# wakensky/parameter_server

Hardware: AMD Instinct MI355X
Metric: aggregated kv-pairs/s (device-resident), N-way sparse push merge at 1/2/4/8 GPU (higher is better)
Workload: dtype f32; 1 GPU; cfg2: 8 pushes x 131072 sorted unique uint64 keys + f32 values, 10% shared keys (U=956,827); 64 such (channel,time) aggregates per GPU per step; global_batch=64, input_layout=arena, parallelism=key-range shards evenDivide(1); worker-sliced ingress, no data-path collective

## Files before the change

include/psg.h:

```cpp
#ifndef PSG_H_
#define PSG_H_

#include <stddef.h>
#include <stdint.h>

#ifdef __cplusplus
extern "C" {
#endif

#define PSG_ABI_VERSION 1
#define PSG_MAX_VALUE_ARRAYS 4

typedef enum psg_status {
  PSG_OK = 0,
  PSG_ERR_ARG = -1,
  PSG_ERR_UNMATCHED = -2,
  PSG_ERR_RANGE = -3,
  PSG_ERR_NO_TIME = -4,
  PSG_ERR_OOM = -5,
  PSG_ERR_DEVICE = -6,
  PSG_ERR_UNSORTED = -7,
  PSG_ERR_SIZE = -8,
  PSG_ERR_CHANNEL = -9,
  PSG_ERR_EMPTY_KEYS = -10,
  PSG_ERR_SIGNATURE = -11
} psg_status;

typedef enum psg_dtype { PSG_F32 = 0, PSG_F64 = 1 } psg_dtype;

#define PSG_SERIAL_MATCH 0u
#define PSG_PARALLEL_MATCH 1u
#define PSG_HOLD_BUFFERS 0x100u
#define PSG_FORM_PACKED 0x1000u
#define PSG_FORM_UNIFORM 0x2000u
#define PSG_PART_SEARCH 0x4000u
#define PSG_PART_STREAM 0x8000u
#define PSG_GROUP32 0x10000u
#define PSG_GROUP64 0x20000u
#define PSG_NO_DENSE 0x40000u
#define PSG_NO_ZERO_COPY 0x80000u
#define PSG_NO_INDEX 0x100000u
#define PSG_FORM_CURSOR 0x400000u
#define PSG_NO_CURSOR 0x800000u
#define PSG_STATIC_KEYS 0x200000u

int psg_abi_version(void);
const char* psg_status_string(int status);
const char* psg_last_error(void);
int psg_device_count(int* n);

typedef struct psg_ctx psg_ctx;

int psg_create(int device, int dtype, unsigned flags, psg_ctx** out);
int psg_destroy(psg_ctx* ctx);
int psg_set_match_flags(psg_ctx* ctx, unsigned flags);
int psg_set_flush_pushes(psg_ctx* ctx, int n);

int psg_key_union(psg_ctx* ctx, int chl, const uint64_t* keys, size_t n);
int psg_key_union_batch(psg_ctx* ctx, int chl, const uint64_t* const* keys, const size_t* n,
                        int npush);
int psg_key_size(psg_ctx* ctx, int chl, size_t* n);
int psg_key_copy(psg_ctx* ctx, int chl, size_t off, size_t n, uint64_t* out);
int psg_find_range(psg_ctx* ctx, int chl, uint64_t kb, uint64_t ke,
                   size_t* lo, size_t* hi);
int psg_value_assign(psg_ctx* ctx, int chl, const void* vals, size_t n);
int psg_value_size(psg_ctx* ctx, int chl, size_t* n);
int psg_value_copy(psg_ctx* ctx, int chl, size_t off, size_t n, void* out);

int psg_push(psg_ctx* ctx, int chl, int time, uint64_t kb, uint64_t ke,
             const uint64_t* keys, size_t n, int m, const void* const* vals);

int psg_push_compressed(psg_ctx* ctx, int chl, int time, uint64_t kb, uint64_t ke,
                        const void* ckeys, size_t ckeys_bytes, int m,
                        const void* const* cvals, const size_t* cvals_bytes);

#define PSG_KC_SIG 1u
// ... 17 lines not shown
                 const uint64_t* keys_dev, size_t n, int m, const void* const* vals_dev,
                 size_t slice, void* stream);
int psg_pull_dev(psg_ctx* ctx, int chl, const uint64_t* keys_dev, size_t n, void* out_dev,
                 unsigned long long* matched_dev, void* stream);
int psg_dev_status(psg_ctx* ctx);

typedef struct psg_merge_job {
  const uint64_t* keys;
  uint64_t nslots;
  int npush;
  const uint64_t* const* push_keys;
  const void* const* push_vals;
  const uint64_t* push_n;
  void* const* out;
} psg_merge_job;

typedef struct psg_plan psg_plan;

int psg_plan_create(int device, int dtype, int m, unsigned flags,
                    const psg_merge_job* jobs, int njobs, psg_plan** out);
int psg_plan_max_push(void);
int psg_plan_run(psg_plan* plan, void* stream);
int psg_plan_run_stage(psg_plan* plan, int stage, void* stream);
int psg_plan_matched(psg_plan* plan, uint64_t* matched);
#define PSG_KERNEL_TILE 0
#define PSG_KERNEL_TILE64 1
#define PSG_KERNEL_PACKED 2
#define PSG_KERNEL_DENSE 3
#define PSG_KERNEL_CURSOR 4
#define PSG_KERNEL_PACKED_CURSOR 5
int psg_plan_form(psg_plan* plan, int* form);
int psg_plan_bytes(psg_plan* plan, uint64_t* bytes, uint64_t* kv_pairs);
int psg_plan_index_info(psg_plan* plan, uint64_t* index_bytes, uint64_t* marked_tiles);
int psg_plan_destroy(psg_plan* plan);

int psg_gather_dev(int dtype, const uint64_t* dkeys, uint64_t nd,
                   const void* dvals, const uint64_t* req, uint64_t nreq,
                   void* out, unsigned long long* matched, void* stream);

int psg_key_union_dev(const uint64_t* a, uint64_t na, const uint64_t* b,
                      uint64_t nb, uint64_t* out, uint64_t* nout,
                      void* stream);

typedef struct psg_nway psg_nway;
int psg_nway_max_push(void);
int psg_nway_create(int device, int dtype, int m, unsigned flags, int npush,
                    const uint64_t* const* keys, const uint64_t* n, const void* const* vals,
                    uint64_t* out_keys, void* const* out_vals, psg_nway** out);
int psg_nway_create_batch(int device, int dtype, int m, unsigned flags, int nmerge,
                          const int* npush, const uint64_t* const* keys, const uint64_t* n,
                          const void* const* vals, uint64_t* const* out_keys,
                          void* const* out_vals, psg_nway** out);
int psg_nway_run(psg_nway* u, void* stream);
int psg_nway_count_dev(psg_nway* u, unsigned long long** nout);
int psg_nway_result(psg_nway* u, uint64_t* nout);
int psg_nway_bytes(psg_nway* u, uint64_t* bytes, uint64_t* kv_pairs);
int psg_nway_destroy(psg_nway* u);

#define PSG_COMM_ID_BYTES 128
typedef struct psg_comm psg_comm;
int psg_comm_unique_id(uint8_t* id);
int psg_comm_init(int device, int nranks, const uint8_t* id, int rank,
                  psg_comm** out);
int psg_comm_destroy(psg_comm* comm);
int psg_comm_init_loopback(int device, int nranks, psg_comm** out);

// ... 205 lines not shown
```

parameter_server_amd/_lib.py:

```python
from __future__ import annotations

import ctypes as C
import os

_HERE = os.path.dirname(os.path.abspath(__file__))
LIB_PATH = os.environ.get("PSG_LIB_PATH") or os.path.join(_HERE, "libpsg.so")

PSG_OK = 0
PSG_ERR_ARG = -1
PSG_ERR_UNMATCHED = -2
PSG_ERR_RANGE = -3
PSG_ERR_NO_TIME = -4
PSG_ERR_OOM = -5
PSG_ERR_DEVICE = -6
PSG_ERR_UNSORTED = -7
PSG_ERR_SIZE = -8
PSG_ERR_CHANNEL = -9
PSG_ERR_EMPTY_KEYS = -10
PSG_ERR_SIGNATURE = -11
PSG_KC_SIG = 1
PSG_KC_KEYS = 2
PSG_KC_ERASE = 4
PSG_MAX_SIG_LEN = 2048
PSG_NO_SLICE = (1 << 64) - 1

PSG_F32 = 0
PSG_F64 = 1
PSG_SERIAL_MATCH = 0
PSG_PARALLEL_MATCH = 1
PSG_HOLD_BUFFERS = 0x100
PSG_FORM_PACKED = 0x1000
PSG_FORM_UNIFORM = 0x2000
PSG_PART_SEARCH = 0x4000
PSG_PART_STREAM = 0x8000
PSG_GROUP32 = 0x10000
PSG_GROUP64 = 0x20000
PSG_NO_DENSE = 0x40000
PSG_NO_ZERO_COPY = 0x80000
PSG_NO_INDEX = 0x100000
PSG_STATIC_KEYS = 0x200000
PSG_FORM_CURSOR = 0x400000
PSG_NO_CURSOR = 0x800000
(PSG_KERNEL_TILE, PSG_KERNEL_TILE64, PSG_KERNEL_PACKED, PSG_KERNEL_DENSE, PSG_KERNEL_CURSOR,
 PSG_KERNEL_PACKED_CURSOR) = range(6)
MAX_VALUE_ARRAYS = 4
MB_STAGES = ("sort", "run_length", "localize", "count_keys", "times", "logit", "trans_times")
PSG_LOSS_LOGIT = 0
(PSG_MB_SORTED_KEY, PSG_MB_SORTED_POS, PSG_MB_UNIQ_KEY, PSG_MB_KEY_CNT, PSG_MB_NEW_OFFSET,
 PSG_MB_NEW_INDEX, PSG_MB_NEW_VALUE, PSG_MB_POS, PSG_MB_NEG, PSG_MB_XW, PSG_MB_TAU, PSG_MB_LOSS,
 PSG_MB_GRAD, PSG_MB_RUN_START, PSG_MB_REMAPPED, PSG_MB_ROW_OF, PSG_MB_SCRATCH) = range(17)
PSG_AUC_BY_KEY, PSG_AUC_AS_WRITTEN = 0, 1
(PSG_MB_DARLING_DUAL, PSG_MB_DARLING_CUR_W, PSG_MB_DARLING_DELTA, PSG_MB_DARLING_ACTIVE,
 PSG_MB_DARLING_DELTA_W) = range(32, 37)
PSG_MB_OFFSET, PSG_MB_INDEX, PSG_MB_VALUE, PSG_MB_Y = range(24, 28)
PSG_TEXT_ADFEA, PSG_TEXT_LIBSVM = 4, 5

_u64 = C.c_uint64
_sz = C.c_size_t
_p = C.c_void_p
_pu64 = C.POINTER(C.c_uint64)
_psz = C.POINTER(C.c_size_t)


class MergeJob(C.Structure):

    _fields_ = [
        ("keys", _p),
        ("nslots", _u64),
        ("npush", C.c_int),
        ("push_keys", C.POINTER(_p)),
        ("push_vals", C.POINTER(_p)),
        ("push_n", _pu64),
        ("out", C.POINTER(_p)),
    ]

# ... 26 lines not shown
    "psg_set_flush_pushes": (C.c_int, [_p, C.c_int]),
    "psg_set_match_flags": (C.c_int, [_p, C.c_uint]),
    "psg_key_union": (C.c_int, [_p, C.c_int, _p, _sz]),
    "psg_key_size": (C.c_int, [_p, C.c_int, _psz]),
    "psg_key_copy": (C.c_int, [_p, C.c_int, _sz, _sz, _p]),
    "psg_find_range": (C.c_int, [_p, C.c_int, _u64, _u64, _psz, _psz]),
    "psg_value_assign": (C.c_int, [_p, C.c_int, _p, _sz]),
    "psg_value_size": (C.c_int, [_p, C.c_int, _psz]),
    "psg_value_copy": (C.c_int, [_p, C.c_int, _sz, _sz, _p]),
    "psg_push": (C.c_int, [_p, C.c_int, C.c_int, _u64, _u64, _p, _sz, C.c_int,
                           C.POINTER(_p)]),
    "psg_push_cached": (C.c_int, [_p, C.c_int, C.c_int, C.c_int, _u64, _u64, C.c_uint,
                                  C.c_uint32, _p, _sz, C.c_int, _p, _sz]),
    "psg_key_cache_clear": (C.c_int, [_p, C.c_int]),
    "psg_push_compressed": (C.c_int, [_p, C.c_int, C.c_int, _u64, _u64, _p, _sz, C.c_int,
                                      _p, _p]),
    "psg_key_cache_bytes": (C.c_int, [_p, C.c_int, _psz]),
    "psg_received_shape": (C.c_int, [_p, C.c_int, C.POINTER(C.c_int), _psz, _psz]),
    "psg_received": (C.c_int, [_p, C.c_int, C.c_int, C.POINTER(_p)]),
    "psg_gather": (C.c_int, [_p, C.c_int, _p, _sz, _p, _psz]),
    "psg_push_dev": (C.c_int, [_p, C.c_int, C.c_int, _u64, _u64, _p, _sz, C.c_int,
                               C.POINTER(_p), _sz, _p]),
    "psg_pull_dev": (C.c_int, [_p, C.c_int, _p, _sz, _p, _p, _p]),
    "psg_dev_status": (C.c_int, [_p]),
    "psg_plan_create": (C.c_int, [C.c_int, C.c_int, C.c_int, C.c_uint,
                                  C.POINTER(MergeJob), C.c_int, C.POINTER(_p)]),
    "psg_plan_max_push": (C.c_int, []),
    "psg_plan_run": (C.c_int, [_p, _p]),
    "psg_plan_run_stage": (C.c_int, [_p, C.c_int, _p]),
    "psg_plan_matched": (C.c_int, [_p, _pu64]),
    "psg_plan_bytes": (C.c_int, [_p, _pu64, _pu64]),
    "psg_plan_form": (C.c_int, [_p, C.POINTER(C.c_int)]),
    "psg_plan_index_info": (C.c_int, [_p, _pu64, _pu64]),
    "psg_plan_destroy": (C.c_int, [_p]),
    "psg_gather_dev": (C.c_int, [C.c_int, _p, _u64, _p, _p, _u64, _p, _p, _p]),
    "psg_key_union_dev": (C.c_int, [_p, _u64, _p, _u64, _p, _pu64, _p]),
    "psg_shard_bounds": (C.c_int, [_sz, _pu64]),
    "psg_slice_dev": (C.c_int, [_p, _u64, _u64, _u64, _p, C.c_int, _p, _p]),
    "psg_crc32c_dev": (C.c_int, [_p, _p, _u64, _u64, _p, _p, _p]),
    "psg_snappy_uncompress_dev": (C.c_int, [_p, _p, _u64, _p, _p, _p, _p]),
    "psg_snappy_uncompressed_length": (C.c_int, [_p, _sz, _psz]),
    "psg_freq_resize": (C.c_int, [_p, C.c_int, C.c_int, C.c_int]),
    "psg_freq_clear": (C.c_int, [_p, C.c_int]),
    "psg_freq_empty": (C.c_int, [_p, C.c_int, C.POINTER(C.c_int)]),
    "psg_freq_insert": (C.c_int, [_p, C.c_int, _p, _p, _sz]),
    "psg_freq_query": (C.c_int, [_p, C.c_int, _p, _sz, C.c_int, _p, _psz]),
    "psg_freq_insert_dev": (C.c_int, [_p, C.c_int, _p, _p, _sz, _p]),
    "psg_freq_query_scratch_bytes": (_sz, [_sz]),
    "psg_freq_query_dev": (C.c_int, [_p, C.c_int, _p, _sz, C.c_int, _p, _p, _p, _p]),
    "psg_freq_table": (C.c_int, [_p, C.c_int, _p, _sz]),
    "psg_freq_table_assign": (C.c_int, [_p, C.c_int, _p, _sz]),
    "psg_comm_unique_id": (C.c_int, [_p]),
    "psg_comm_init": (C.c_int, [C.c_int, C.c_int, _p, C.c_int, C.POINTER(_p)]),
    "psg_comm_destroy": (C.c_int, [_p]),
    "psg_comm_init_loopback": (C.c_int, [C.c_int, C.c_int, C.POINTER(_p)]),
    "psg_exchange_create": (C.c_int, [_p, C.c_int, C.c_int, C.c_int, _p, _p, _p,
                                      C.POINTER(_p)]),
    "psg_exchange_run": (C.c_int, [_p, _p]),
    "psg_exchange_recv": (C.c_int, [_p, C.POINTER(_p), _p, _pu64, _p, _pu64]),
    "psg_exchange_destroy": (C.c_int, [_p]),
    "psg_exchange_status": (C.c_int, [_p, _pu64]),
    "psg_exchange_create_local": (C.c_int, [C.c_int, C.c_int, C.c_int, C.c_int, C.c_int, _p,
                                            _p, _p, C.POINTER(_p)]),
    "psg_exchange_set_direct": (C.c_int, [_p, C.c_int]),
    "psg_exchange_send_layout": (C.c_int, [_p, C.POINTER(_p), _p, _p]),
    "psg_key_union_batch": (C.c_int, [_p, C.c_int, _p, _p, C.c_int]),
# ... 120 lines not shown
```

parameter_server_amd/csrc/psg_internal.h:

```cpp
#pragma once

#include <hip/hip_runtime.h>
#include <stdint.h>

namespace psg {

constexpr int kMaxPush = 4096;
constexpr int kMaxM = 4;
constexpr int kTileSlots = 1024;
#ifndef PSG_PACK_TS
#define PSG_PACK_TS 2048
#endif
constexpr int kPackTileSlots = PSG_PACK_TS;
constexpr int kWideSlots = 2048;

constexpr uint32_t kFlagParallel = 1u;
constexpr uint32_t kFlagCont = 2u;
constexpr uint32_t kFlagLastTile = 4u;

enum PartMode : uint32_t { kSearch = 0, kStream = 1 };
constexpr uint32_t kStreamChunk = 512;

struct JobDev {
  const uint64_t* dkeys;
// ... 28 lines not shown
  const uint64_t* dpos;
  const uint32_t* bt;
};

struct CursorJob {
  const uint64_t* dkeys;
  uint64_t nslots;
  const uint64_t* const* pkeys;
  const void* const* pvals;
  const uint64_t* pn;
  void* const* out;
  unsigned long long* fail;
  uint32_t* seg;
  const uint32_t* bt;
  uint32_t np, ntiles, flags;
  uint32_t kr;
};
struct CursorChunk {
  uint32_t job, t0, t1;
};
constexpr int kCursorPushes = 32;
hipError_t launch_aggregate_cursor(int dtype, int m, int kr, const CursorJob* d_jobs,
                                   const CursorChunk* d_chunks, uint32_t nchunks, uint32_t* bx,
                                   hipStream_t stream);

struct DenseCheck {
  const uint64_t* keys;
  uint64_t n;
  const uint64_t* D;
  uint64_t nd;
  unsigned long long* out;
};

hipError_t launch_partition(const JobDev* d_jobs, const uint32_t* d_split_item_job,
                            uint32_t nsplit_items, const uint64_t* d_items,
                            uint32_t nitems, hipStream_t stream, bool xcd = false);
hipError_t launch_aggregate_tile(int dtype, int m, const TileDesc* d_tiles, uint32_t ntiles,
                                 int form, hipStream_t stream);
uint32_t bucket_index_words(uint32_t tile_slots);
hipError_t launch_bucket_index(const TileDesc* d_tiles, uint32_t ntiles, uint32_t tile_slots,
                               uint32_t* out, unsigned long long* nmarked,
                               hipStream_t stream);
constexpr int kPackCursorPushes = 256;
hipError_t launch_aggregate_tile_packed(int dtype, int m, const TileDesc* d_tiles,
                                        uint32_t ntiles, hipStream_t stream,
                                        const CursorChunk* d_chunks = nullptr,
                                        uint32_t nchunks = 0, uint32_t* bx = nullptr);
hipError_t launch_aggregate_dense(int dtype, int m, const TileDesc* d_tiles, uint32_t ntiles,
                                  hipStream_t stream);
hipError_t launch_dense_check(const DenseCheck* checks, uint32_t nchecks, const uint64_t* items,
                              uint64_t nitems, hipStream_t stream);
hipError_t launch_gather(int dtype, const uint64_t* dkeys, uint64_t nd,
                         const void* dvals, const uint64_t* req, uint64_t nreq,
                         void* out, unsigned long long* matched,
                         hipStream_t stream);
hipError_t launch_pull(int dtype, const uint64_t* dkeys, uint64_t nd, const void* dvals,
                       const uint64_t* req, uint64_t nreq, void* out, unsigned long long* matched,
                       unsigned long long* ctl, unsigned long long* unsorted_total,
                       hipStream_t stream);
struct IntakeArgs {
  const void* src[kMaxM + 1];
  void* dst[kMaxM + 1];
  uint64_t len[kMaxM + 1];
  uint32_t esz[kMaxM + 1];
  uint32_t n = 0;
  const uint64_t* claim_keys = nullptr;
  const uint64_t* D = nullptr;
  uint64_t nclaim = 0;
  unsigned long long* bad = nullptr;
// ... 137 lines not shown
```

parameter_server_amd/csrc/psg_jobimage.cc:

```cpp
#include "psg_jobimage.h"

#include <algorithm>
#include <cmath>
#include <cstring>

#include "psg_host.h"

namespace psg {
namespace {

constexpr double kStreamBelow = 24.0;
constexpr double kPackBelow = 16.0;


uint64_t search_groups(uint64_t nt) { return (nt + 64) / 64; }
uint64_t stream_chunks(uint64_t n) { return (n + kStreamChunk - 1) / kStreamChunk; }
uint64_t split_blocks(uint64_t nt, uint64_t np) { return (std::max(nt + 1, np) + 255) / 256; }

}

int JobImage::plan(const JobSpec* jobs, size_t njobs, int dt, int mm, bool idx) {
  if (njobs > (1ull << 27)) return fail(PSG_ERR_ARG, "too many jobs");
  dtype = dt;
  m = mm;
// ... 132 lines not shown
  L.marked = off;
  if (use_index()) off += 256;
  L.sitems = off;
  off = align_up(off + 4 * (size_t)nsplit, 256);
  L.items = off;
  off = align_up(off + 8 * (size_t)nitems, 256);
  L.cjobs = off;
  if (cursor) off = align_up(off + sizeof(CursorJob) * njobs, 256);
  L.chunks = off;
  if (chunked) off = align_up(off + sizeof(CursorChunk) * nchunks, 256);
  L.zero = off;
  size_t fail_cur = off;
  uint64_t npall = 0;
  for (const JobInfo& I : info) npall += I.np;
  off = align_up(off + 8 * npall, 256);
  L.bx = off;
  if (chunked) off = align_up(off + 4 * (size_t)bxs * ((size_t)nchunks + 1), 256);
  L.zero_end = off;
  L.job.resize(njobs);
  for (size_t j = 0; j < njobs; ++j) {
    const size_t np = info[j].np, nt = info[j].ntiles;
    JobLayout::Job& o = L.job[j];
    o.pk = off; off = align_up(off + 8 * np, 64);
    o.pv = off; off = align_up(off + 8 * np * m, 64);
    o.pn = off; off = align_up(off + 8 * np, 64);
    o.out = off; off = align_up(off + 8 * m, 64);
    o.fail = fail_cur; fail_cur += 8 * np;
    o.seg = off; off = align_up(off + 4 * (nt + 1) * np, 256);
    o.split = off;
    if (info[j].has_split) off = align_up(off + 8 * (nt + 1), 256);
    o.dpos = off;
    if (jobs[j].dense) off = align_up(off + 8 * np, 256);
  }
  L.total = off;
}

bool JobImage::same_shape(const JobSpec* jobs, const void* base) {
  shape.clear();
  if (index || cursor || pcursor) return false;
  const JobLayout& L = lay;
  shape.insert(shape.end(), {(uint64_t)h.size(), tile, (uint64_t)m, (uint64_t)dtype,
                             (uint64_t)pack, (uint64_t)wide, (uint64_t)(uintptr_t)base, L.total,
                             L.tiles, L.zero, nitems, nsplit, ntiles});
  for (size_t j = 0; j < h.size(); ++j) {
    const JobSpec& s = jobs[j];
    const JobDev& d = h[j];
    const JobLayout::Job& o = L.job[j];
    shape.insert(shape.end(), {(uint64_t)info[j].np, s.nslots, (uint64_t)(uintptr_t)s.keys,
                               (uint64_t)s.flags, (uint64_t)s.dense, (uint64_t)d.mode,
                               (uint64_t)d.segq, (uint64_t)d.segb, o.pk, o.pv, o.pn, o.out,
                               o.fail, o.seg, o.split, o.dpos});
    if (d.mode == kStream) shape.insert(shape.end(), info[j].pn.begin(), info[j].pn.end());
  }
  return shape == last_shape;
}

void JobImage::keep_shape() {
  last_shape.swap(shape);
  shape.clear();
}

int JobImage::fill(const JobSpec* jobs, char* img, const void* dev, bool same) {
  const JobLayout& L = lay;
  char* base = (char*)dev;
  const size_t njobs = h.size();
  if (L.zero_end > L.zero) memset(img + L.zero, 0, L.zero_end - L.zero);
  if (use_index()) memset(img + L.marked, 0, 8);
  TileDesc* htiles = (TileDesc*)(img + L.tiles);
  uint32_t* hsitems = (uint32_t*)(img + L.sitems);
  uint64_t* hitems = (uint64_t*)(img + L.items);
  const uint32_t* bt = use_index() ? (const uint32_t*)(base + L.index) : nullptr;
  uint64_t tcur = 0, icur = 0, scur = 0;
  for (size_t j = 0; j < njobs; ++j) {
    const JobSpec& s = jobs[j];
    JobInfo& I = info[j];
    const JobLayout::Job& o = L.job[j];
    const uint32_t np = I.np, nt = I.ntiles;
    uint64_t* hk = (uint64_t*)(img + o.pk);
    uint64_t* hv = (uint64_t*)(img + o.pv);
    for (uint32_t p = 0; p < np; ++p) {
      const uint32_t c = I.slot[p];
      hk[p] = (uint64_t)s.pkeys[c];
      for (int i = 0; i < m; ++i) hv[(size_t)p * m + i] = (uint64_t)s.pvals[(size_t)c * m + i];
    }
    if (np) memcpy(img + o.pn, I.pn.data(), 8 * np);
    if (s.dense) {
      uint64_t* hd = (uint64_t*)(img + o.dpos);
      uint32_t* hs = (uint32_t*)(img + o.seg);
      for (uint32_t p = 0; p < np; ++p) {
        const uint64_t dp = s.dpos[I.slot[p]], n = I.pn[p];
        hd[p] = dp;
        for (uint32_t t = 0; t <= nt; ++t) {
          const uint64_t edge = (uint64_t)t * tile;
          const uint64_t v = edge <= dp ? 0 : std::min<uint64_t>(edge - dp, n);
          hs[(size_t)t * np + p] = (uint32_t)v;
        }
      }
    }
    memcpy(img + o.out, s.out.data(), 8 * m);
    JobDev& d = h[j];
    d.dkeys = s.keys;
    d.pkeys = (const uint64_t* const*)(base + o.pk);
    d.pn = (const uint64_t*)(base + o.pn);
    d.seg = (uint32_t*)(base + o.seg);
    d.fail = (unsigned long long*)(base + o.fail);
    d.split = I.has_split ? (uint64_t*)(base + o.split) : nullptr;
    I.seg = d.seg;
    I.fail = d.fail;
    if (same) continue;
    for (uint32_t b = 0; b < I.nsplit; ++b) hsitems[scur++] = (uint32_t)j;
    if (I.nitems && d.mode == kSearch) {
      const uint64_t ng = search_groups(nt);
      for (uint64_t g = 0; g < ng; ++g)
        for (uint32_t p = 0; p < np; ++p)
          hitems[icur++] = (uint64_t)j << 37 | (uint64_t)p << 24 | g;
    } else if (I.nitems) {
      for (uint32_t p = 0; p < np; ++p) {
        const uint64_t nc = stream_chunks(I.pn[p]);
        for (uint64_t c = 0; c < nc; ++c)
          hitems[icur++] = (uint64_t)j << 37 | (uint64_t)p << 24 | c;
      }
    }
    for (uint32_t t = 0; t < nt; ++t) {
      TileDesc& T = htiles[tcur];
      const uint64_t slot0 = (uint64_t)t * tile;
      T.dk = s.keys + slot0;
      T.seg = d.seg + (size_t)t * d.segb;
      T.pkeys = d.pkeys;
      T.pvals = (const void* const*)(base + o.pv);
      T.pn = d.pn;
      T.out = (void* const*)(base + o.out);
      T.fail = d.fail;
      T.slot0 = slot0;
// ... 53 lines not shown
```

parameter_server_amd/csrc/psg_jobimage.h:

```cpp
#pragma once

#include <stddef.h>
#include <stdint.h>
#include <vector>

#include "psg_internal.h"

namespace psg {

inline size_t align_up(size_t x, size_t a) { return (x + a - 1) / a * a; }

struct JobSpec {
  const uint64_t* keys;
  uint64_t nslots;
  std::vector<const uint64_t*> pkeys;
  std::vector<const void*> pvals;
  std::vector<uint64_t> pn;
  std::vector<void*> out;
  uint32_t flags;
  bool dense = false;
  std::vector<uint64_t> dpos;
};

struct JobInfo {
  uint32_t np = 0, ntiles = 0;
  std::vector<uint64_t> pn;
  std::vector<uint32_t> slot;
  uint32_t ncaller = 0;
  uint32_t* seg = nullptr;
  uint32_t segq = 1;
  unsigned long long* fail = nullptr;
  uint32_t kr = 0;
  uint32_t nch = 0, ch0 = 0;
  uint32_t nitems = 0, nsplit = 0;
  bool has_split = false;
};

struct JobLayout {
  static constexpr size_t jobs = 0;
  size_t tiles = 0;
  size_t index = 0;
  size_t marked = 0;
  size_t sitems = 0;
  size_t items = 0;
  size_t cjobs = 0;
  size_t chunks = 0;
  size_t zero = 0, bx = 0, zero_end = 0;
  struct Job { size_t pk, pv, pn, out, fail, seg, split, dpos; };
  std::vector<Job> job;
  size_t total = 0;
  uint32_t iw = 0;
};

struct JobImage {
  int knob_part = -1, knob_pack = -1, knob_wide = -1, knob_cursor = -1;

  int dtype = 0, m = 1;
  bool index = false;
  bool pack = false;
  bool wide = false;
  bool dense = false;
  bool cursor = false;
  bool pcursor = false;
  uint32_t tile = kTileSlots;
  uint32_t bxs = 32;
  uint32_t nchunks = 0;
  uint32_t ckr = 3;
  uint32_t ntiles = 0, nitems = 0, nsplit = 0;
  bool all_search = false;
  std::vector<JobDev> h;
  std::vector<JobInfo> info;
  JobLayout lay;
  bool use_index() const { return index && !dense; }

  std::vector<uint64_t> last_shape, shape;

  int plan(const JobSpec* jobs, size_t njobs, int dtype, int m, bool index);
  void layout(const JobSpec* jobs, uint32_t iw);
  bool same_shape(const JobSpec* jobs, const void* base);
  void keep_shape();
  int fill(const JobSpec* jobs, char* img, const void* base, bool same);
};

}
```

parameter_server_amd/csrc/psg_jobtable.h:

```cpp
#pragma once

#include <hip/hip_runtime.h>
#include <vector>

#include "psg_jobimage.h"

namespace psg {

int detect_dense(std::vector<JobSpec>& specs);

struct JobTable : JobImage {
  int device = -1;
  void read_knobs(unsigned flags);
  bool split_once = false;
  uint64_t index_bytes = 0, marked_tiles = 0;
  void* blob = nullptr;
  size_t blob_bytes = 0;
  JobDev* d_jobs = nullptr;
  TileDesc* d_tiles = nullptr;
  uint32_t* d_split_items = nullptr;
  uint64_t* d_items = nullptr;
  CursorJob* d_cjobs = nullptr;
  CursorChunk* d_chunks = nullptr;
  uint32_t* d_bx = nullptr;
  void* d_zero = nullptr;
  size_t zero_bytes = 0;
  char* himg[2] = {nullptr, nullptr};
  const void* himg_dev[2] = {nullptr, nullptr};
  bool zero_copy = true;
  size_t himg_cap[2] = {0, 0};
  hipEvent_t himg_ev[2] = {nullptr, nullptr};
  int himg_cur = 0;

  void release();
  int build(int dev, int dtype, int m, const std::vector<JobSpec>& jobs,
            hipStream_t strm = nullptr, bool async = false, bool index = false);
  int run_stage(int stage, hipStream_t s) const;
  int run(hipStream_t s) const;
  int matched(std::vector<uint64_t>& out) const;

 private:
  void release_blob();
  int ensure_memory(int ib, hipStream_t strm, bool async);
  int upload(int ib, bool same, hipStream_t strm);
};

}
```

parameter_server_amd/csrc/psg_jobtable.hip:

```cpp
#include "psg_jobtable.h"

#include <utility>

#include "psg_host.h"

namespace psg {

int detect_dense(std::vector<JobSpec>& specs) {
  std::vector<DenseCheck> hc;
  std::vector<std::pair<size_t, size_t>> at;
  std::vector<uint64_t> items;
  for (size_t j = 0; j < specs.size(); ++j) {
    const JobSpec& s = specs[j];
    if (s.nslots == 0) continue;
    for (size_t p = 0; p < s.pn.size(); ++p) {
      if (s.pn[p] == 0) continue;
      if (s.pn[p] > s.nslots) goto next_job;
      at.emplace_back(j, p);
      hc.push_back(DenseCheck{s.pkeys[p], s.pn[p], s.keys, s.nslots, nullptr});
    }
  next_job:;
  }
  if (hc.empty()) return PSG_OK;
  for (size_t c = 0; c < hc.size(); ++c)
// ... 98 lines not shown
    cb.d[0] = HostCopyDesc{himg_dev[ib], blob, (uint64_t)head};
    cb.d[1] = HostCopyDesc{(const char*)himg_dev[ib] + tail, base + tail, (uint64_t)(total - tail)};
    HIP_TRY(launch_host_copy_batch(cb, strm));
  } else if (same) {
    HIP_TRY(hipMemcpyAsync(blob, img, head, hipMemcpyHostToDevice, strm));
    HIP_TRY(hipMemcpyAsync(base + tail, img + tail, total - tail, hipMemcpyHostToDevice, strm));
  } else if (zc_ok) {
    HIP_TRY(launch_host_copy(blob, himg_dev[ib], total, strm));
  } else {
    HIP_TRY(hipMemcpyAsync(blob, img, total, hipMemcpyHostToDevice, strm));
  }
  return PSG_OK;
}

int JobTable::build(int dev, int dt, int mm, const std::vector<JobSpec>& jobs, hipStream_t strm,
                    bool async, bool idx) {
  device = dev;
  if (int rc = plan(jobs.data(), jobs.size(), dt, mm, idx)) return rc;
  layout(jobs.data(), bucket_index_words(tile));
  const int ib = himg_cur;
  himg_cur ^= 1;
  if (int rc = ensure_memory(ib, strm, async)) return rc;
  const bool same = same_shape(jobs.data(), blob);
  if (int rc = fill(jobs.data(), himg[ib], blob, same)) return rc;
  char* base = (char*)blob;
  const bool chunked = cursor || pcursor;
  d_jobs = (JobDev*)blob;
  d_tiles = (TileDesc*)(base + lay.tiles);
  d_split_items = (uint32_t*)(base + lay.sitems);
  d_items = (uint64_t*)(base + lay.items);
  d_cjobs = cursor ? (CursorJob*)(base + lay.cjobs) : nullptr;
  d_chunks = chunked ? (CursorChunk*)(base + lay.chunks) : nullptr;
  d_bx = chunked ? (uint32_t*)(base + lay.bx) : nullptr;
  d_zero = base + lay.zero;
  zero_bytes = lay.zero_end - lay.zero;
  if (int rc = upload(ib, same, strm)) return rc;
  keep_shape();
  HIP_TRY(hipEventRecord(himg_ev[ib], strm));
  index_bytes = 0;
  marked_tiles = 0;
  unsigned long long* d_marked = (unsigned long long*)(base + lay.marked);
  if (use_index())
    HIP_TRY(launch_bucket_index(d_tiles, ntiles, tile, (uint32_t*)(base + lay.index), d_marked,
                                strm));
  split_once = index && nsplit > 0 && !dense && !chunked;
  if (split_once)
    HIP_TRY(launch_partition(d_jobs, d_split_items, nsplit, nullptr, 0, strm));
  if (!async) HIP_TRY(hipStreamSynchronize(strm));
  if (use_index()) {
    index_bytes = 4 * (uint64_t)lay.iw * ntiles;
    if (ntiles) {
      HIP_TRY(hipMemcpyAsync(&marked_tiles, d_marked, 8, hipMemcpyDeviceToHost, strm));
      HIP_TRY(hipStreamSynchronize(strm));
    }
  }
  return PSG_OK;
}

int JobTable::run_stage(int stage, hipStream_t s) const {
  if (h.empty()) return PSG_OK;
  if (stage == 0) {
    if (cursor || pcursor)
      HIP_TRY(hipMemsetAsync(d_zero, 0, zero_bytes, s));
    else if (!dense)
      HIP_TRY(launch_partition(d_jobs, d_split_items, split_once ? 0u : nsplit, d_items, nitems, s,
                               all_search));
  } else if (cursor)
    HIP_TRY(launch_aggregate_cursor(dtype, m, (int)ckr, d_cjobs, d_chunks, nchunks, d_bx, s));
  else if (dense)
    HIP_TRY(launch_aggregate_dense(dtype, m, d_tiles, ntiles, s));
  else if (pack)
    HIP_TRY(launch_aggregate_tile_packed(dtype, m, d_tiles, ntiles, s,
                                         pcursor ? d_chunks : nullptr, nchunks, d_bx));
  else
    HIP_TRY(launch_aggregate_tile(dtype, m, d_tiles, ntiles, wide ? 1 : 0, s));
  return PSG_OK;
}

int JobTable::run(hipStream_t s) const {
  if (int rc = run_stage(0, s)) return rc;
  return run_stage(1, s);
}

int JobTable::matched(std::vector<uint64_t>& out) const {
  out.clear();
  for (size_t j = 0; j < h.size(); ++j) {
    const JobInfo& I = info[j];
    std::vector<uint64_t> mt(I.ncaller, 0);
    const uint32_t np = I.np, nt = I.ntiles;
    if (np && nt) {
      std::vector<unsigned long long> f(np);
      std::vector<uint32_t> first(np), last(np);
      const size_t pitch = 4 * (size_t)I.segq;
      const size_t segb = I.segq == 1 ? np : 1;
      HIP_TRY(hipMemcpy(f.data(), I.fail, 8 * np, hipMemcpyDeviceToHost));
      HIP_TRY(hipMemcpy2D(first.data(), 4, I.seg, pitch, 4, np, hipMemcpyDeviceToHost));
      HIP_TRY(hipMemcpy2D(last.data(), 4, I.seg + (size_t)nt * segb, pitch, 4, np,
                          hipMemcpyDeviceToHost));
      std::vector<uint32_t> bxw;
// ... 22 lines not shown
```

parameter_server_amd/csrc/psg_partition.hip:

```cpp
#include <hip/hip_runtime.h>
#include <stdint.h>

#include "psg_device.h"
#include "psg_internal.h"

namespace psg {

namespace {

__device__ __forceinline__ uint32_t uni(uint32_t v) { return __builtin_amdgcn_readfirstlane(v); }
__device__ __forceinline__ uint64_t uni64(uint64_t v) {
  return ((uint64_t)uni((uint32_t)(v >> 32)) << 32) | uni((uint32_t)v);
}

__global__ __launch_bounds__(256) void splitter_kernel(const JobDev* __restrict__ jobs,
                                                       const uint32_t* __restrict__ item_job,
                                                       uint32_t nitems) {
  const uint32_t item = blockIdx.x;
  if (item >= nitems) return;
  const uint32_t j = uni(item_job[item]);
  const JobDev& J = jobs[j];
  const uint32_t first = uni(J.split_begin);
  const uint64_t t = (uint64_t)(item - first) * 256u + threadIdx.x;
  if (t < J.ntiles) J.split[t] = J.dkeys[t * J.tile];
  if (t == J.ntiles) J.split[t] = J.dkeys[J.nslots - 1] + 1ull;
  if (t < J.npush) J.fail[t] = 0ull;
}

using dev::bracket_lower_bound;

__device__ __forceinline__ void search_item(const JobDev& J, uint32_t p, uint32_t g, int lane) {
  const uint32_t b = (g << 6) + (uint32_t)lane;
  const bool valid = b <= J.ntiles;
  const uint64_t* S = J.pkeys[p];
  const uint64_t n = J.pn[p];
  const uint32_t bc = valid ? b : J.ntiles;
  const bool up = bc == J.ntiles;
  const uint64_t xl = J.split ? J.split[bc]
                      : up ? J.dkeys[J.nslots - 1] + 1ull : J.dkeys[(uint64_t)bc * J.tile];
  const uint64_t k0 = S[0], kn = S[n - 1];
  const int last = (int)((J.ntiles - (g << 6)) < 63u ? (J.ntiles - (g << 6)) : 63u);
  const bool edge = (lane & 15) == 0 || lane == last;
  const int lo_l = lane & ~15;
  const int hi_l = lo_l + 16 < last ? lo_l + 16 : last;
  uint64_t res = 0;
  if (edge) {
    res = xl <= k0 ? 0 : (xl > kn ? n : bracket_lower_bound(S, xl, 0, n - 1, k0, kn));
  }
  const uint64_t r0 = (uint64_t)__shfl((long long)res, lo_l, 64);
  const uint64_t r1 = (uint64_t)__shfl((long long)res, hi_l, 64);
  if (!edge) {
    if (xl <= k0) {
      res = 0;
    } else if (xl > kn) {
      res = n;
    } else {
      uint64_t a = r0 > 0 ? r0 - 1 : 0, c = r1 < n ? r1 : n - 1;
      uint64_t ka = 0, kc = 0;
      bool ok = a < c;
      if (ok) {
        ka = S[a];
        kc = S[c];
        ok = ka < xl && xl <= kc;
      }
      res = ok ? bracket_lower_bound(S, xl, a, c, ka, kc) : bracket_lower_bound(S, xl, 0, n - 1, k0, kn);
    }
  }
  if (valid) {
    J.seg[(size_t)p * J.segq + (size_t)b * J.segb] = (uint32_t)res;
    if (b == 0) J.fail[p] = 0ull;
  }
}

constexpr uint32_t kKPL = kStreamChunk / 64;
__device__ __forceinline__ void stream_item(const JobDev& J, uint32_t p, uint32_t c, int lane,
                                            uint64_t* ck ) {
  const uint64_t* S = J.pkeys[p];
  const uint64_t n = J.pn[p];
  const uint32_t nt = J.ntiles;
  const __attribute__((address_space(1))) uint64_t* sp =
      (const __attribute__((address_space(1))) uint64_t*)J.split;
  __attribute__((address_space(1))) uint32_t* seg =
      (__attribute__((address_space(1))) uint32_t*)(J.seg + (size_t)p * J.segq);
  const uint64_t i0 = (uint64_t)c * kStreamChunk;
  const uint32_t cl = (uint32_t)(n - i0 < kStreamChunk ? n - i0 : kStreamChunk);
  const bool last = i0 + cl == n;
  uint64_t k[kKPL];
  const __attribute__((address_space(1))) uint64_t* Sg =
      (const __attribute__((address_space(1))) uint64_t*)(S + i0);
#pragma unroll
  for (int j = 0; j < kKPL; ++j) {
    const uint32_t x = 64u * j + (uint32_t)lane;
    k[j] = x < cl ? Sg[x] : ~0ull;
  }
  int64_t T0 = -1;
  int64_t g = 0;
  uint64_t w0 = ~0ull, w1 = ~0ull;
  int32_t win = -1;
  if (i0 > 0) {
    int64_t gq = (int64_t)((double)i0 / (double)n * (double)nt) - 32;
    gq = gq + 128 > (int64_t)nt + 1 ? (int64_t)nt + 1 - 128 : gq;
    gq = gq < 0 ? 0 : gq;
    const int64_t tq = gq + lane;
// ... 39 lines not shown
  __builtin_amdgcn_wave_barrier();
  __builtin_amdgcn_fence(__ATOMIC_ACQUIRE, "wavefront");
  const uint64_t klast = uni64(ck[cl - 1]);
  for (int64_t t0 = T0 + 1; t0 <= (int64_t)nt; t0 += 64) {
    const int64_t t = t0 + lane;
    uint64_t sv;
    if (win >= 0) {
      const int32_t x = win + lane;
      const uint64_t a0 = (uint64_t)__shfl((long long)w0, x & 63, 64);
      const uint64_t a1 = (uint64_t)__shfl((long long)w1, x & 63, 64);
      sv = t <= (int64_t)nt ? (x < 64 ? a0 : a1) : ~0ull;
      win = -1;
    } else {
      sv = t <= (int64_t)nt ? sp[t] : ~0ull;
    }
    uint32_t pos = 0;
#pragma unroll
    for (uint32_t st = kStreamChunk / 2; st > 0; st >>= 1)
      if (pos + st <= cl && ck[pos + st - 1] < sv) pos += st;
    pos += (pos < cl && ck[pos] < sv) ? 1u : 0u;
    if (t <= (int64_t)nt && (pos < cl || last)) seg[t] = (uint32_t)(i0 + pos);
    if (!last && uni64((uint64_t)__shfl((long long)sv, 63, 64)) > klast) break;
  }
  if (c == 0 && lane == 0) J.fail[p] = 0ull;
}

__device__ __forceinline__ uint32_t xcd_block(uint32_t b, uint32_t n) {
  const uint32_t x = b & 7u, j = b >> 3, q = n >> 3, r = n & 7u;
  return x * q + (x < r ? x : r) + j;
}

__global__ __launch_bounds__(256) void partition_kernel(const JobDev* __restrict__ jobs,
                                                        const uint64_t* __restrict__ items,
                                                        uint32_t nitems, int xcd) {
  __shared__ uint64_t ck[4][kStreamChunk];
  const uint32_t blk = xcd ? xcd_block(blockIdx.x, gridDim.x) : blockIdx.x;
  const uint32_t item = uni((blk * 256u + threadIdx.x) >> 6);
  const int lane = threadIdx.x & 63;
  if (item >= nitems) return;
  const uint64_t it = uni64(items[item]);
  const uint32_t j = (uint32_t)(it >> 37);
  const uint32_t p = (uint32_t)(it >> 24) & 0x1fffu;
  const uint32_t x = (uint32_t)it & 0xffffffu;
  const JobDev& J = jobs[j];
  if (J.mode == kStream)
    stream_item(J, p, x, lane, ck[threadIdx.x >> 6]);
  else
    search_item(J, p, x, lane);
}

}

hipError_t launch_partition(const JobDev* d_jobs, const uint32_t* d_split_item_job,
                            uint32_t nsplit_items, const uint64_t* d_items, uint32_t nitems,
                            hipStream_t stream, bool xcd) {
  if (nsplit_items)
    hipLaunchKernelGGL(splitter_kernel, dim3(nsplit_items), dim3(256), 0, stream, d_jobs,
                       d_split_item_job, nsplit_items);
  if (nitems)
    hipLaunchKernelGGL(partition_kernel, dim3((nitems + 3) / 4), dim3(256), 0, stream, d_jobs,
                       d_items, nitems, xcd ? 1 : 0);
  return hipGetLastError();
}

}
```

parameter_server_amd/csrc/psg_plan.hip:

```cpp
#include "psg_ctx.h"

struct psg_plan {
  JobTable table;
  hipStream_t last = nullptr;
  uint64_t bytes = 0, kv = 0;
};

extern "C" {

int psg_plan_max_push(void) { return psg::kMaxPush; }

int psg_plan_create(int device, int dtype, int m, unsigned flags,
                    const psg_merge_job* jobs, int njobs, psg_plan** out) {
  if (!out || (njobs > 0 && !jobs)) return fail(PSG_ERR_ARG, "null argument");
  if (dtype != PSG_F32 && dtype != PSG_F64) return fail(PSG_ERR_ARG, "dtype %d", dtype);
  if (m < 1 || m > PSG_MAX_VALUE_ARRAYS) return fail(PSG_ERR_ARG, "m=%d", m);
  if (int rc = set_dev(device)) return rc;
  std::vector<JobSpec> specs(njobs);
  uint64_t bytes = 0, kv = 0;
  const uint64_t sv = vsize(dtype);
  for (int j = 0; j < njobs; ++j) {
    const psg_merge_job& J = jobs[j];
    if (J.npush < 0 || (J.npush > 0 && (!J.push_keys || !J.push_vals || !J.push_n)) ||
        !J.out || (J.nslots > 0 && !J.keys))
      return fail(PSG_ERR_ARG, "job %d: null pointer", j);
    JobSpec& s = specs[j];
    s.keys = J.keys;
    s.nslots = J.nslots;
    s.flags = (flags & PSG_PARALLEL_MATCH) ? psg::kFlagParallel : 0u;
    for (int p = 0; p < J.npush; ++p) {
      s.pkeys.push_back(J.push_keys[p]);
      for (int i = 0; i < m; ++i) s.pvals.push_back(J.push_vals[(size_t)p * m + i]);
      s.pn.push_back(J.push_n[p]);
      bytes += J.push_n[p] * (8 + m * sv);
      kv += J.push_n[p];
    }
    for (int i = 0; i < m; ++i) s.out.push_back(J.out[i]);
    bytes += J.nslots * (8 + m * sv);
  }
  if ((flags & PSG_STATIC_KEYS) && !(flags & PSG_NO_DENSE))
    if (int rc = detect_dense(specs)) return rc;
  psg_plan* p = new psg_plan();
  p->table.read_knobs(flags);
  int rc = p->table.build(device, dtype, m, specs, nullptr, false, !(flags & PSG_NO_INDEX));
  if (rc) {
    p->table.release();
    delete p;
    return rc;
  }
  p->bytes = bytes;
  p->kv = kv;
  *out = p;
  return PSG_OK;
}

int psg_plan_run(psg_plan* plan, void* stream) {
  if (!plan) return fail(PSG_ERR_ARG, "null plan");
  plan->last = (hipStream_t)stream;
  return plan->table.run((hipStream_t)stream);
}

int psg_plan_run_stage(psg_plan* plan, int stage, void* stream) {
  if (!plan || stage < 0 || stage > 1) return fail(PSG_ERR_ARG, "bad plan/stage");
  plan->last = (hipStream_t)stream;
  return plan->table.run_stage(stage, (hipStream_t)stream);
}

int psg_plan_matched(psg_plan* plan, uint64_t* matched) {
  if (!plan || !matched) return fail(PSG_ERR_ARG, "null argument");
  if (int rc = set_dev(plan->table.device)) return rc;
  HIP_TRY(hipStreamSynchronize(plan->last));
  std::vector<uint64_t> mt;
  if (int rc = plan->table.matched(mt)) return rc;
  std::copy(mt.begin(), mt.end(), matched);
  return PSG_OK;
}

int psg_plan_form(psg_plan* plan, int* form) {
  if (!plan || !form) return fail(PSG_ERR_ARG, "null argument");
  const JobTable& T = plan->table;
  *form = T.cursor ? PSG_KERNEL_CURSOR
          : T.pcursor ? PSG_KERNEL_PACKED_CURSOR
          : T.dense ? PSG_KERNEL_DENSE
          : T.pack  ? PSG_KERNEL_PACKED
          : T.wide  ? PSG_KERNEL_TILE64
                    : PSG_KERNEL_TILE;
  return PSG_OK;
}

int psg_plan_index_info(psg_plan* plan, uint64_t* index_bytes, uint64_t* marked_tiles) {
  if (!plan) return fail(PSG_ERR_ARG, "null plan");
  if (index_bytes) *index_bytes = plan->table.index_bytes;
  if (marked_tiles) *marked_tiles = plan->table.marked_tiles;
  return PSG_OK;
}

int psg_plan_bytes(psg_plan* plan, uint64_t* bytes, uint64_t* kv) {
  if (!plan) return fail(PSG_ERR_ARG, "null plan");
  if (bytes) *bytes = plan->bytes;
  if (kv) *kv = plan->kv;
  return PSG_OK;
}

int psg_plan_destroy(psg_plan* plan) {
  if (!plan) return PSG_OK;
  (void)hipSetDevice(plan->table.device);
  plan->table.release();
  delete plan;
  return PSG_OK;
}

int psg_gather_dev(int dtype, const uint64_t* dkeys, uint64_t nd,
                   const void* dvals, const uint64_t* req, uint64_t nreq,
                   void* out, unsigned long long* matched, void* stream) {
  if (dtype != PSG_F32 && dtype != PSG_F64) return fail(PSG_ERR_ARG, "dtype");
  HIP_TRY(psg::launch_gather(dtype, dkeys, nd, dvals, req, nreq, out, matched,
                             (hipStream_t)stream));
  return PSG_OK;
}

int psg_key_union_dev(const uint64_t* a, uint64_t na, const uint64_t* b,
                      uint64_t nb, uint64_t* out, uint64_t* nout, void* stream) {
  if (!out || !nout || (na && !a) || (nb && !b)) return fail(PSG_ERR_ARG, "null");
  if (na + nb >= (1ull << 32)) return fail(PSG_ERR_ARG, "na + nb >= 2^32");
  hipStream_t s = (hipStream_t)stream;
  std::vector<const uint64_t*> pk;
// ... 76 lines not shown
```

parameter_server_amd/kv_vector.py:

```python
from __future__ import annotations

import ctypes as C
from dataclasses import dataclass, field
from typing import List, Optional, Sequence

import numpy as np

from . import _lib
from ._lib import PSG_F32, PSG_F64, PSG_PARALLEL_MATCH, PSG_SERIAL_MATCH

KEY_ALL = (0, (1 << 64) - 1)


def _np_dtype(dtype: int):
    return np.float32 if dtype == PSG_F32 else np.float64


def _ptr(a: np.ndarray) -> int:
    return a.ctypes.data


@dataclass
class Message:

# ... 175 lines not shown
            pn = (C.c_uint64 * max(1, npush))(*J["push_n"])
            out = _lib.ptr_array(J["out"])
            self._keep += [pk, pv, pn, out]
            cj[j].keys = J["keys"]
            cj[j].nslots = J["nslots"]
            cj[j].npush = npush
            cj[j].push_keys = C.cast(pk, C.POINTER(C.c_void_p))
            cj[j].push_vals = C.cast(pv, C.POINTER(C.c_void_p))
            cj[j].push_n = C.cast(pn, C.POINTER(C.c_uint64))
            cj[j].out = C.cast(out, C.POINTER(C.c_void_p))
        h = C.c_void_p()
        flags = (flags & ~PSG_PARALLEL_MATCH) | (PSG_PARALLEL_MATCH if parallel_match
                                                 else PSG_SERIAL_MATCH)
        _lib.check(self._L.psg_plan_create(device, dtype, m, flags, cj, len(jobs),
                                           C.byref(h)))
        self._h = h
        self.npush_total = sum(len(J["push_keys"]) for J in jobs)
        b, kv = C.c_uint64(), C.c_uint64()
        _lib.check(self._L.psg_plan_bytes(h, C.byref(b), C.byref(kv)))
        self.bytes, self.kv_pairs = b.value, kv.value
        f = C.c_int()
        _lib.check(self._L.psg_plan_form(h, C.byref(f)))
        self.form = f.value
        ib, mt = C.c_uint64(), C.c_uint64()
        _lib.check(self._L.psg_plan_index_info(h, C.byref(ib), C.byref(mt)))
        self.index_bytes, self.marked_tiles = ib.value, mt.value

    def run(self, stream: Optional[int] = None) -> None:
        _lib.check(self._L.psg_plan_run(self._h, stream or None))

    def run_stage(self, stage: int, stream: Optional[int] = None) -> None:
        _lib.check(self._L.psg_plan_run_stage(self._h, stage, stream or None))

    def matched(self) -> np.ndarray:
        out = np.zeros(max(1, self.npush_total), np.uint64)
        _lib.check(self._L.psg_plan_matched(
            self._h, out.ctypes.data_as(C.POINTER(C.c_uint64))))
        return out[: self.npush_total]

    def close(self):
        if getattr(self, "_h", None):
            self._L.psg_plan_destroy(self._h)
            self._h = None

    def __del__(self):
        try:
            self.close()
        except Exception:
            pass


class NWayMergeBatch:

    def __init__(self, device: int, dtype: int, merges, parallel_match: bool = False):
        self._L = _lib.lib()
        m = len(merges[0]["out_vals"]) if merges else 0
        npush = [len(x["push_keys"]) for x in merges]
        keys = [k for x in merges for k in x["push_keys"]]
        ns = [n for x in merges for n in x["push_n"]]
        vals = [v for x in merges for vs in x["push_vals"] for v in vs]
        np_ = (C.c_int * max(1, len(npush)))(*npush)
        pk = _lib.ptr_array(keys) if keys else None
        pn = (C.c_uint64 * max(1, len(ns)))(*ns)
        pv = _lib.ptr_array(vals) if m and vals else None
        ok = _lib.ptr_array([x["out_keys"] for x in merges])
        ov = _lib.ptr_array([v for x in merges for v in x["out_vals"]]) if m else None
# ... 78 lines not shown
```

Baseline: 184.3 billion kv-pairs/s.

## Warm-start partition search from previous run's boundaries with per-item hint state

```diff
diff --git a/include/psg.h b/include/psg.h
--- a/include/psg.h
+++ b/include/psg.h
@@ -42,6 +42,7 @@
 #define PSG_NO_INDEX 0x100000u
 #define PSG_FORM_CURSOR 0x400000u
 #define PSG_NO_CURSOR 0x800000u
+#define PSG_NO_HINTS 0x1000000u
 #define PSG_STATIC_KEYS 0x200000u
 
 int psg_abi_version(void);
@@ -125,6 +126,7 @@
 int psg_plan_form(psg_plan* plan, int* form);
 int psg_plan_bytes(psg_plan* plan, uint64_t* bytes, uint64_t* kv_pairs);
 int psg_plan_index_info(psg_plan* plan, uint64_t* index_bytes, uint64_t* marked_tiles);
+int psg_plan_hint_state(psg_plan* plan, uint64_t counts[4]);
 int psg_plan_destroy(psg_plan* plan);
 
 int psg_gather_dev(int dtype, const uint64_t* dkeys, uint64_t nd,
diff --git a/parameter_server_amd/_lib.py b/parameter_server_amd/_lib.py
--- a/parameter_server_amd/_lib.py
+++ b/parameter_server_amd/_lib.py
@@ -41,6 +41,7 @@
 PSG_STATIC_KEYS = 0x200000
 PSG_FORM_CURSOR = 0x400000
 PSG_NO_CURSOR = 0x800000
+PSG_NO_HINTS = 0x1000000
 (PSG_KERNEL_TILE, PSG_KERNEL_TILE64, PSG_KERNEL_PACKED, PSG_KERNEL_DENSE, PSG_KERNEL_CURSOR,
  PSG_KERNEL_PACKED_CURSOR) = range(6)
 MAX_VALUE_ARRAYS = 4
@@ -133,6 +134,7 @@
     "psg_plan_bytes": (C.c_int, [_p, _pu64, _pu64]),
     "psg_plan_form": (C.c_int, [_p, C.POINTER(C.c_int)]),
     "psg_plan_index_info": (C.c_int, [_p, _pu64, _pu64]),
+    "psg_plan_hint_state": (C.c_int, [_p, _pu64]),
     "psg_plan_destroy": (C.c_int, [_p]),
     "psg_gather_dev": (C.c_int, [C.c_int, _p, _u64, _p, _p, _u64, _p, _p, _p]),
     "psg_key_union_dev": (C.c_int, [_p, _u64, _p, _u64, _p, _pu64, _p]),
diff --git a/parameter_server_amd/csrc/psg_internal.h b/parameter_server_amd/csrc/psg_internal.h
--- a/parameter_server_amd/csrc/psg_internal.h
+++ b/parameter_server_amd/csrc/psg_internal.h
@@ -84,9 +84,11 @@
   unsigned long long* out;
 };
 
+enum : uint32_t { kHintSearched = 0, kHintOff = 1, kHintKept = 2, kHintFresh = 3 };
 hipError_t launch_partition(const JobDev* d_jobs, const uint32_t* d_split_item_job,
                             uint32_t nsplit_items, const uint64_t* d_items,
-                            uint32_t nitems, hipStream_t stream, bool xcd = false);
+                            uint32_t nitems, hipStream_t stream, bool xcd = false,
+                            uint32_t* hstate = nullptr);
 hipError_t launch_aggregate_tile(int dtype, int m, const TileDesc* d_tiles, uint32_t ntiles,
                                  int form, hipStream_t stream);
 uint32_t bucket_index_words(uint32_t tile_slots);
diff --git a/parameter_server_amd/csrc/psg_jobimage.cc b/parameter_server_amd/csrc/psg_jobimage.cc
--- a/parameter_server_amd/csrc/psg_jobimage.cc
+++ b/parameter_server_amd/csrc/psg_jobimage.cc
@@ -188,6 +188,8 @@
     o.dpos = off;
     if (jobs[j].dense) off = align_up(off + 8 * np, 256);
   }
+  L.hstate = off;
+  if (hints) off = align_up(off + 4 * (size_t)nitems, 256);
   L.total = off;
 }
 
@@ -222,6 +224,8 @@
   const size_t njobs = h.size();
   if (L.zero_end > L.zero) memset(img + L.zero, 0, L.zero_end - L.zero);
   if (use_index()) memset(img + L.marked, 0, 8);
+  if (hints)
+    for (uint32_t i = 0; i < nitems; ++i) ((uint32_t*)(img + L.hstate))[i] = kHintFresh;
   TileDesc* htiles = (TileDesc*)(img + L.tiles);
   uint32_t* hsitems = (uint32_t*)(img + L.sitems);
   uint64_t* hitems = (uint64_t*)(img + L.items);
@@ -255,6 +259,8 @@
     }
     memcpy(img + o.out, s.out.data(), 8 * m);
     JobDev& d = h[j];
+    if (hints && nt && !s.dense && d.mode == kSearch)
+      memset(img + o.seg, 0, 4 * ((size_t)nt + 1) * np);
     d.dkeys = s.keys;
     d.pkeys = (const uint64_t* const*)(base + o.pk);
     d.pn = (const uint64_t*)(base + o.pn);
diff --git a/parameter_server_amd/csrc/psg_jobimage.h b/parameter_server_amd/csrc/psg_jobimage.h
--- a/parameter_server_amd/csrc/psg_jobimage.h
+++ b/parameter_server_amd/csrc/psg_jobimage.h
@@ -48,6 +48,7 @@
   size_t zero = 0, bx = 0, zero_end = 0;
   struct Job { size_t pk, pv, pn, out, fail, seg, split, dpos; };
   std::vector<Job> job;
+  size_t hstate = 0;
   size_t total = 0;
   uint32_t iw = 0;
 };
@@ -68,6 +69,7 @@
   uint32_t ckr = 3;
   uint32_t ntiles = 0, nitems = 0, nsplit = 0;
   bool all_search = false;
+  bool hints = false;
   std::vector<JobDev> h;
   std::vector<JobInfo> info;
   JobLayout lay;
diff --git a/parameter_server_amd/csrc/psg_jobtable.h b/parameter_server_amd/csrc/psg_jobtable.h
--- a/parameter_server_amd/csrc/psg_jobtable.h
+++ b/parameter_server_amd/csrc/psg_jobtable.h
@@ -23,6 +23,7 @@
   CursorJob* d_cjobs = nullptr;
   CursorChunk* d_chunks = nullptr;
   uint32_t* d_bx = nullptr;
+  uint32_t* d_hstate = nullptr;
   void* d_zero = nullptr;
   size_t zero_bytes = 0;
   char* himg[2] = {nullptr, nullptr};
diff --git a/parameter_server_amd/csrc/psg_jobtable.hip b/parameter_server_amd/csrc/psg_jobtable.hip
--- a/parameter_server_amd/csrc/psg_jobtable.hip
+++ b/parameter_server_amd/csrc/psg_jobtable.hip
@@ -154,6 +154,7 @@
   d_cjobs = cursor ? (CursorJob*)(base + lay.cjobs) : nullptr;
   d_chunks = chunked ? (CursorChunk*)(base + lay.chunks) : nullptr;
   d_bx = chunked ? (uint32_t*)(base + lay.bx) : nullptr;
+  d_hstate = hints && nitems ? (uint32_t*)(base + lay.hstate) : nullptr;
   d_zero = base + lay.zero;
   zero_bytes = lay.zero_end - lay.zero;
   if (int rc = upload(ib, same, strm)) return rc;
@@ -186,7 +187,7 @@
       HIP_TRY(hipMemsetAsync(d_zero, 0, zero_bytes, s));
     else if (!dense)
       HIP_TRY(launch_partition(d_jobs, d_split_items, split_once ? 0u : nsplit, d_items, nitems, s,
-                               all_search));
+                               all_search, d_hstate));
   } else if (cursor)
     HIP_TRY(launch_aggregate_cursor(dtype, m, (int)ckr, d_cjobs, d_chunks, nchunks, d_bx, s));
   else if (dense)
diff --git a/parameter_server_amd/csrc/psg_partition.hip b/parameter_server_amd/csrc/psg_partition.hip
--- a/parameter_server_amd/csrc/psg_partition.hip
+++ b/parameter_server_amd/csrc/psg_partition.hip
@@ -29,27 +29,42 @@
 
 using dev::bracket_lower_bound;
 
-__device__ __forceinline__ void search_item(const JobDev& J, uint32_t p, uint32_t g, int lane) {
+
+__device__ __forceinline__ void search_item(const JobDev& J, uint32_t p, uint32_t g, int lane,
+                                            uint32_t* ws) {
+  const uint32_t st = ws ? uni(*ws) : 0u;
+  const bool test = ws && (st == kHintSearched || st == kHintKept);
   const uint32_t b = (g << 6) + (uint32_t)lane;
   const bool valid = b <= J.ntiles;
   const uint64_t* S = J.pkeys[p];
   const uint64_t n = J.pn[p];
   const uint32_t bc = valid ? b : J.ntiles;
   const bool up = bc == J.ntiles;
+  uint32_t* sg = J.seg + ((size_t)p * J.segq + (size_t)bc * J.segb);
+  const uint64_t old = ws && st != kHintFresh ? (uint64_t)*sg : ~0ull;
   const uint64_t xl = J.split ? J.split[bc]
                       : up ? J.dkeys[J.nslots - 1] + 1ull : J.dkeys[(uint64_t)bc * J.tile];
   const uint64_t k0 = S[0], kn = S[n - 1];
+  const bool inb = test && old <= n;
+  const uint64_t kl = inb && old > 0 ? S[old - 1] : 0ull;
+  const uint64_t kh = inb && old < n ? S[old] : 0ull;
+  const bool hit = inb && (old == 0 || kl < xl) && (old == n || kh >= xl);
+  if (test && __all(hit)) {
+    if (valid && b == 0) J.fail[p] = 0ull;
+    if (st != kHintKept && lane == 0) *ws = kHintKept;
+    return;
+  }
   const int last = (int)((J.ntiles - (g << 6)) < 63u ? (J.ntiles - (g << 6)) : 63u);
   const bool edge = (lane & 15) == 0 || lane == last;
   const int lo_l = lane & ~15;
   const int hi_l = lo_l + 16 < last ? lo_l + 16 : last;
-  uint64_t res = 0;
-  if (edge) {
+  uint64_t res = hit ? old : 0;
+  if (edge && !hit) {
     res = xl <= k0 ? 0 : (xl > kn ? n : bracket_lower_bound(S, xl, 0, n - 1, k0, kn));
   }
   const uint64_t r0 = (uint64_t)__shfl((long long)res, lo_l, 64);
   const uint64_t r1 = (uint64_t)__shfl((long long)res, hi_l, 64);
-  if (!edge) {
+  if (!edge && !hit) {
     if (xl <= k0) {
       res = 0;
     } else if (xl > kn) {
@@ -67,8 +82,18 @@
     }
   }
   if (valid) {
-    J.seg[(size_t)p * J.segq + (size_t)b * J.segb] = (uint32_t)res;
+    if (!hit) *sg = (uint32_t)res;
     if (b == 0) J.fail[p] = 0ull;
+  }
+  if (ws) {
+    uint32_t nw = kHintSearched;
+    if (test) {
+      const uint32_t missed = (uint32_t)__popcll(__ballot(valid && !hit));
+      nw = 2u * missed > (uint32_t)last + 1u ? kHintOff : kHintSearched;
+    } else if (st == kHintOff) {
+      nw = __all(!valid || res == old) ? kHintSearched : kHintOff;
+    }
+    if (nw != st && lane == 0) *ws = nw;
   }
 }
 
@@ -174,7 +199,7 @@
 
 __global__ __launch_bounds__(256) void partition_kernel(const JobDev* __restrict__ jobs,
                                                         const uint64_t* __restrict__ items,
-                                                        uint32_t nitems, int xcd) {
+                                                        uint32_t nitems, int xcd, uint32_t* hstate) {
   __shared__ uint64_t ck[4][kStreamChunk];
   const uint32_t blk = xcd ? xcd_block(blockIdx.x, gridDim.x) : blockIdx.x;
   const uint32_t item = uni((blk * 256u + threadIdx.x) >> 6);
@@ -188,20 +213,20 @@
   if (J.mode == kStream)
     stream_item(J, p, x, lane, ck[threadIdx.x >> 6]);
   else
-    search_item(J, p, x, lane);
+    search_item(J, p, x, lane, hstate ? hstate + item : nullptr);
 }
 
 }
 
 hipError_t launch_partition(const JobDev* d_jobs, const uint32_t* d_split_item_job,
                             uint32_t nsplit_items, const uint64_t* d_items, uint32_t nitems,
-                            hipStream_t stream, bool xcd) {
+                            hipStream_t stream, bool xcd, uint32_t* hstate) {
   if (nsplit_items)
     hipLaunchKernelGGL(splitter_kernel, dim3(nsplit_items), dim3(256), 0, stream, d_jobs,
                        d_split_item_job, nsplit_items);
   if (nitems)
     hipLaunchKernelGGL(partition_kernel, dim3((nitems + 3) / 4), dim3(256), 0, stream, d_jobs,
-                       d_items, nitems, xcd ? 1 : 0);
+                       d_items, nitems, xcd ? 1 : 0, hstate);
   return hipGetLastError();
 }
 
diff --git a/parameter_server_amd/csrc/psg_plan.hip b/parameter_server_amd/csrc/psg_plan.hip
--- a/parameter_server_amd/csrc/psg_plan.hip
+++ b/parameter_server_amd/csrc/psg_plan.hip
@@ -42,6 +42,7 @@
     if (int rc = detect_dense(specs)) return rc;
   psg_plan* p = new psg_plan();
   p->table.read_knobs(flags);
+  p->table.hints = !(flags & PSG_NO_HINTS);
   int rc = p->table.build(device, dtype, m, specs, nullptr, false, !(flags & PSG_NO_INDEX));
   if (rc) {
     p->table.release();
@@ -92,6 +93,22 @@
   if (!plan) return fail(PSG_ERR_ARG, "null plan");
   if (index_bytes) *index_bytes = plan->table.index_bytes;
   if (marked_tiles) *marked_tiles = plan->table.marked_tiles;
+  return PSG_OK;
+}
+
+int psg_plan_hint_state(psg_plan* plan, uint64_t counts[4]) {
+  if (!plan || !counts) return fail(PSG_ERR_ARG, "null argument");
+  const JobTable& T = plan->table;
+  for (int i = 0; i < 4; ++i) counts[i] = 0;
+  if (!T.d_hstate) return PSG_OK;
+  if (int rc = set_dev(T.device)) return rc;
+  HIP_TRY(hipStreamSynchronize(plan->last));
+  std::vector<uint32_t> st(T.nitems);
+  HIP_TRY(hipMemcpy(st.data(), T.d_hstate, 4 * (size_t)T.nitems, hipMemcpyDeviceToHost));
+  size_t i = 0;
+  for (size_t j = 0; j < T.h.size(); ++j)
+    for (uint32_t k = 0; k < T.info[j].nitems; ++k, ++i)
+      if (T.h[j].mode == psg::kSearch) counts[st[i] & 3u]++;
   return PSG_OK;
 }
 
diff --git a/parameter_server_amd/kv_vector.py b/parameter_server_amd/kv_vector.py
--- a/parameter_server_amd/kv_vector.py
+++ b/parameter_server_amd/kv_vector.py
@@ -231,6 +231,11 @@
     def run_stage(self, stage: int, stream: Optional[int] = None) -> None:
         _lib.check(self._L.psg_plan_run_stage(self._h, stage, stream or None))
 
+    def hint_state(self) -> List[int]:
+        c = (C.c_uint64 * 4)()
+        _lib.check(self._L.psg_plan_hint_state(self._h, c))
+        return list(c)
+
     def matched(self) -> np.ndarray:
         out = np.zeros(max(1, self.npush_total), np.uint64)
         _lib.check(self._L.psg_plan_matched(
```

Measured after the change: 199.5 billion kv-pairs/s, median of 6. 8.2% higher.
